# tum-vision/skeletondiffusion

Measured on AMD Instinct MI355X. Metric: generated futures/sec (AMASS 16-joint, 50 futures, T=100) at 1/2/4/8 GPUs, higher is better.
Workload: dtype f32 (emulated: 3 x f16 split products); 1 GPU; AMASS 16-joint nonisotropic sampling, T=100, 50 futures, batch=64 (config 2); J=16, T=100, sequences_per_gpu=64, sequences_total=64, futures=50, rows_per_gpu=3200, latent_dim=96, hipgraph=True, parallelism=dp1 (sequence-sharded, no data-path collective), row_chains=3, route=tiled split (k_gl4t + k_gl4 MODE 2/3), route_bits=24, kernel_variant=0

## Files before the change

### skeletondiffusion_amd/build.py

```python
from __future__ import annotations

import os
import shutil
import subprocess
import sys

HERE = os.path.dirname(os.path.abspath(__file__))
CSRC = os.path.join(HERE, "csrc")
OUT = os.path.join(HERE, "libskeldiff.so")
SOURCES = ["sd_kernels.hip", "sd_graph_linear.hip", "sd_graph_linear_v3.hip", "sd_graph_linear_v4.hip", "sd_graph_linear_v5.hip",
           "sd_metrics.hip", "sd_realism.hip", "sd_fid.hip", "sd_mmgt.hip", "sd_decoder.hip", "sd_train.hip", "sd_gru_train.hip",
           "sd_optim.hip", "sd_motion_batch.hip", "sd_q_sample.hip", "sd_plan.hip"]
HEADERS = ["sd_internal.h", "sd_gl4_args.h", "sd_realism_addr.h", "sd_gru_gates.h", "sd_optim_math.h", "sd_optim_table.h",
           "sd_philox.h", "sd_motion_batch_addr.h", "sd_q_sample_addr.h",
           os.path.join("..", "..", "include", "skeldiff.h")]


def _hipcc() -> str:
    for cand in (os.environ.get("HIPCC"), shutil.which("hipcc"), "/opt/rocm/bin/hipcc"):
        if cand and os.path.exists(cand):
            return cand
    raise RuntimeError("hipcc not found")


def _stale(stamp: str) -> bool:
    if not os.path.exists(OUT) or not os.path.exists(OUT + ".flags"):
        return True
    with open(OUT + ".flags") as f:
        if f.read() != stamp:
            return True
    t = os.path.getmtime(OUT)
    return any(os.path.getmtime(os.path.join(CSRC, f)) > t for f in SOURCES + HEADERS)


DEVICE_FLAGS = ["-Xclang", "-target-feature", "-Xclang", "-packed-fp32-ops"]
_FEATURE_NOTE = b"'-packed-fp32-ops' is not a recognized feature for this target"


def build_library(force: bool = False, verbose: bool = False, extra=(), tag="_dbg",
                  packed_fp32: bool = False) -> str:
    variant = bool(extra) or packed_fp32
    if packed_fp32 and tag == "_dbg":
        tag = "_packed"
    out = OUT.replace(".so", tag + ".so") if variant else OUT
    flags = ["--offload-arch=gfx950", "-O3", "-std=c++17", "-fPIC", "-Wno-pass-failed"] + \
        ([] if packed_fp32 else DEVICE_FLAGS) + list(extra)
    stamp = " ".join(flags)
# ... 45 lines not shown
```

### skeletondiffusion_amd/csrc/sd_graph_linear_v4.hip

```cpp
#include <hip/hip_runtime.h>
#include <stdint.h>

#include <algorithm>
#include <cmath>

#include "sd_gl4_args.h"
#include "sd_internal.h"

namespace sd {

typedef float floatx4 __attribute__((ext_vector_type(4)));
typedef float floatx8 __attribute__((ext_vector_type(8)));
typedef float floatx16 __attribute__((ext_vector_type(16)));
typedef _Float16 halfx8 __attribute__((ext_vector_type(8)));
typedef __bf16 bf16x8 __attribute__((ext_vector_type(8)));
typedef __bf16 bf16x4 __attribute__((ext_vector_type(4)));

namespace {

typedef __attribute__((address_space(3))) void lds_void;

template <int N>
struct VmCnt4 {
    static_assert(N >= 0 && N < 64, "vmcnt range");
    static constexpr int imm = (N & 0xF) | (0x7 << 4) | (0xF << 8) | ((N >> 4) << 14);
};

__device__ __forceinline__ floatx4 g4(const float* p) { return *reinterpret_cast<const floatx4*>(p); }

__device__ __forceinline__ float tanh4(float x) {
    const float e = __builtin_amdgcn_exp2f(2.0f * 1.44269504088896341f * x);
    return 1.0f - 2.0f * __builtin_amdgcn_rcpf(e + 1.0f);
}

__device__ __forceinline__ int64_t blk_off(int64_t row, int node, int f, int J, int F) {
    return ((((row >> 5) * J + node) * (int64_t)F) << 5) + ((f >> 3) << 8) + (((f >> 2) & 1) << 7) +
           ((row & 31) << 2) + (f & 3);
}


__global__ void k_absmax(const float* __restrict__ w, int64_t n, unsigned* __restrict__ out) {
    unsigned m = 0;
    for (int64_t i = (int64_t)blockIdx.x * blockDim.x + threadIdx.x; i < n; i += (int64_t)gridDim.x * blockDim.x)
        m = max(m, __float_as_uint(fabsf(w[i])));
    for (int o = 32; o > 0; o >>= 1) m = max(m, (unsigned)__shfl_xor((int)m, o));
    if ((threadIdx.x & 63) == 0) atomicMax(out, m);
}

__global__ void k_split_w(const float* __restrict__ W, int ntypes, int N, int K, int nct, float scale,
                          _Float16* __restrict__ out) {
    const int nchunk = K >> 4;
    const int64_t total = (int64_t)ntypes * nchunk * nct * 64;
    for (int64_t g = (int64_t)blockIdx.x * blockDim.x + threadIdx.x; g < total; g += (int64_t)gridDim.x * blockDim.x) {
// ... 75 lines not shown
    out->nct = ((N + 31) / 32 + 5) / 6 * 6;
    const int64_t n = (int64_t)ntypes * N * K;
    unsigned* dmax = nullptr;
    unsigned hmax = 0;
    hipError_t e = hipMalloc(&dmax, sizeof(unsigned));
    if (e != hipSuccess) return e;
    if ((e = hipMemsetAsync(dmax, 0, sizeof(unsigned), s)) != hipSuccess) return e;
    hipLaunchKernelGGL(k_absmax, dim3(256), dim3(256), 0, s, W, n, dmax);
    if ((e = hipGetLastError()) != hipSuccess) return e;
    if ((e = hipMemcpyAsync(&hmax, dmax, sizeof(unsigned), hipMemcpyDeviceToHost, s)) != hipSuccess) return e;
    if ((e = hipStreamSynchronize(s)) != hipSuccess) return e;
    (void)hipFree(dmax);
    const float amax = __builtin_bit_cast(float, hmax);
    int ex = 0;
    if (amax > 0.f && amax == amax && amax < 3.0e38f) (void)frexpf(amax, &ex);
    out->scale = ldexpf(1.0f, 15 - ex);
    out->unscale = ldexpf(1.0f, ex - 15);
    const size_t halves = (size_t)ntypes * (K / 16) * out->nct * 1024;
    if ((e = hipMalloc(&out->w, halves * sizeof(_Float16))) != hipSuccess) return e;
    const int64_t total = (int64_t)ntypes * (K / 16) * out->nct * 64;
    const int blocks = (int)std::min<int64_t>((total + 255) / 256, 4096);
    hipLaunchKernelGGL(k_split_w, dim3(blocks), dim3(256), 0, s, W, ntypes, N, K, out->nct, out->scale, out->w);
    return hipGetLastError();
}

struct YDst {
    float* y;
    int64_t y_rs, y_js, y_ts, y_cs;
};
struct YOut {
    GL4GArgs g;
};
static_assert(sizeof(YOut) == sizeof(GL4GArgs), "YOut: the GEMM-phase block");
__device__ __forceinline__ int64_t zs_off(int64_t row, int j, int n, int J, int N) {
    return ((((row >> 5) * (N >> 5) + (n >> 5)) * J + j) << 10) + ((row & 31) << 5) + (n & 31);
}

__device__ __forceinline__ floatx16 exact_tile_f32_impl(const float* x1, int64_t x1_rs, int K1, int x1_div,
                                                                  int64_t x1_row0, int x1_blk, const float* x2,
                                                                  int64_t x2_rs, int K2, int x2_blk, int64_t B, int J,
                                                                  const float* W, int wrow, int N, float unscale,
                                                                  int64_t row0, int j, int col0) {
    const int lane = threadIdx.x & 63, l32 = lane & 31, h = lane >> 5;
    const int K = K1 + K2;
    const int col = col0 + l32;
    const float* wr = W + (int64_t)(wrow + (col < N ? col : 0)) * K + 4 * h;
    const int64_t row = row0 + l32, ac = row < B ? row : 0;
    const float* xr1 = x1 + (x1_blk ? blk_off(row, j, 4 * h, J, K1) : ((ac + x1_row0) / x1_div) * x1_rs + (int64_t)j * K1 + 4 * h);
    const float* xr2 = !K2 ? xr1 : x2 + (x2_blk ? blk_off(row, j, 4 * h, J, K2) : ac * x2_rs + (int64_t)j * K2 + 4 * h);
    floatx16 c;
#pragma unroll
    for (int e = 0; e < 16; ++e) c[e] = 0.f;
#pragma nounroll
    for (int k0 = 0; k0 < K; k0 += 8) {
        const float* xp = k0 < K1 ? xr1 + (x1_blk ? (k0 >> 3) * 256 : k0) : xr2 + (x2_blk ? ((k0 - K1) >> 3) * 256 : k0 - K1);
        const float4 xv = *reinterpret_cast<const float4*>(xp);
        float4 wv = *reinterpret_cast<const float4*>(wr + k0);
        if (col >= N) wv = float4{0.f, 0.f, 0.f, 0.f};
        c = __builtin_amdgcn_mfma_f32_32x32x2f32(xv.x, wv.x, c, 0, 0, 0);
        c = __builtin_amdgcn_mfma_f32_32x32x2f32(xv.y, wv.y, c, 0, 0, 0);
        c = __builtin_amdgcn_mfma_f32_32x32x2f32(xv.z, wv.z, c, 0, 0, 0);
        c = __builtin_amdgcn_mfma_f32_32x32x2f32(xv.w, wv.w, c, 0, 0, 0);
    }
    const float up = 1.0f / unscale;
#pragma unroll
    for (int e = 0; e < 16; ++e) c[e] *= up;
    return c;
}
__device__ __forceinline__ floatx16 exact_tile_f32(const GLArgs& p, int64_t row0, int j, int col0) {
    return exact_tile_f32_impl(p.x1, p.x1_rs, p.K1, p.x1_div, p.x1_row0, p.x1_blk, p.x2, p.x2_rs, p.K2, p.x2_blk, p.B,
                               p.J, p.W, p.wrow[j], p.N, p.wsp_unscale, row0, j, col0);
}

__device__ __forceinline__ void gl4g_preload(const GL4GArgs& p) {
    asm volatile("" ::"s"(p.da.d), "s"(p.da.m), "s"(p.db.d), "s"(p.db.m), "s"(p.q8), "s"(p.r8), "s"(p.J), "s"(p.N), "s"(p.wsp),
                 "s"(p.x1), "s"(p.x2), "s"(p.bias), "s"(p.B), "s"(p.ntile_r), "s"(p.K1), "s"(p.K2), "s"(p.wsp_nct), "s"(p.pair_n),
                 "s"((int)p.x1_blk), "s"((int)p.x2_blk), "s"(p.x1_div));
    asm volatile("" ::"s"(p.ntype4[0]), "s"(p.ntype4[1]), "s"(p.ntype4[2]), "s"(p.ntype4[3]), "s"(p.ntype4[4]), "s"(p.ntype4[5]),
                 "s"(p.ntype4[6]), "s"(p.ntype4[7]), "s"(p.ntype4[8]), "s"(p.ntype4[9]), "s"(p.ntype4[10]), "s"(p.ntype4[11]),
                 "s"(p.ntype4[12]), "s"(p.ntype4[13]), "s"(p.ntype4[14]), "s"(p.ntype4[15]));
}

template <bool RMS, int PREC, bool ROWMAJOR, int PF = 8>
__global__ __launch_bounds__(256) void k_gl4y(const GL4GArgs p) {
    gl4g_preload(p);
    const int lane = threadIdx.x & 63, l32 = lane & 31, h = lane >> 5;
    const int wave = __builtin_amdgcn_readfirstlane(threadIdx.x >> 6);
    const Unit3 un = decode_unit(blockIdx.x * 4u + (uint32_t)wave, p.da, p.db);
    const int tc = (int)un.lo, j = (int)un.mid;
    const int64_t tr = un.hi;
    const int J = p.J;
    if (tr >= p.ntile_r) return;
    const int jt = gl4_node_type(p, j);
    const int64_t row0 = tr * 32;
    const int K = p.K1 + p.K2;
// ... 9 lines not shown

    floatx4 xa[PF], xb[PF];
    halfx8 wh[PF], wl[PF];
    auto issue = [&](int c, int sl) {
        const int k0 = c << 4;
        const float* src;
        int step4;
        if (k0 < p.K1) {
            src = p.x1_blk ? x1r + (k0 << 5) : x1r + k0;
            step4 = p.x1_blk ? 128 : 4;
        } else {
            src = p.x2_blk ? x2r + ((k0 - p.K1) << 5) : x2r + (k0 - p.K1);
            step4 = p.x2_blk ? 128 : 4;
        }
        xa[sl] = g4(src);
        xb[sl] = g4(src + step4);
        const _Float16* w = wbase + c * wcs;
        wh[sl] = *reinterpret_cast<const halfx8*>(w);
        if constexpr (!PREC) wl[sl] = *reinterpret_cast<const halfx8*>(w + 512);
    };
    floatx16 acc;
#pragma unroll
    for (int e = 0; e < 16; ++e) acc[e] = 0.f;
    float ss = 0.f, amx = 0.f;
    auto compute = [&](int c, int sl) {
        const floatx8 f = {xa[sl].x, xa[sl].y, xa[sl].z, xa[sl].w, xb[sl].x, xb[sl].y, xb[sl].z, xb[sl].w};
        if (RMS && (c << 4) < p.K1) {
            const floatx8 q = f * f;
            ss += ((q[0] + q[1]) + (q[2] + q[3])) + ((q[4] + q[5]) + (q[6] + q[7]));
        }
        const floatx8 a = __builtin_elementwise_abs(f);
        amx = fmaxf(amx, fmaxf(fmaxf(fmaxf(a[0], a[1]), fmaxf(a[2], a[3])), fmaxf(fmaxf(a[4], a[5]), fmaxf(a[6], a[7]))));
        const halfx8 xh = __builtin_convertvector(f, halfx8);
        acc = __builtin_amdgcn_mfma_f32_32x32x16_f16(xh, wh[sl], acc, 0, 0, 0);
        if constexpr (!PREC) {
            const halfx8 xl = __builtin_convertvector(f - __builtin_convertvector(xh, floatx8), halfx8);
            acc = __builtin_amdgcn_mfma_f32_32x32x16_f16(xh, wl[sl], acc, 0, 0, 0);
            acc = __builtin_amdgcn_mfma_f32_32x32x16_f16(xl, wh[sl], acc, 0, 0, 0);
        }
    };
    const int ncol = tc * 32 + l32;
    const float bv = (p.bias && ncol < p.N) ? p.bias[jt * p.N + ncol] : 0.f;
#pragma unroll
    for (int i = 0; i < PF; ++i) issue(i, i);
    for (int c0 = 0; c0 < nchunk - PF; c0 += PF) {
#pragma unroll
        for (int i = 0; i < PF; ++i) {
            compute(c0 + i, i);
            issue(c0 + i + PF, i);
        }
    }
#pragma unroll
    for (int i = 0; i < PF; ++i) compute(nchunk - PF + i, i);
    const bool oor = __builtin_amdgcn_ballot_w64(arow < p.B && amx >= 65504.0f) != 0;
    float sc[16];
#pragma unroll
    for (int r = 0; r < 16; ++r) sc[r] = p.wsp_unscale;
    if (RMS) {
        const float t = ss + __shfl_xor(ss, 32);
#pragma unroll
        for (int r = 0; r < 16; ++r) {
            const float n2 = __shfl(t, (r & 3) + 8 * (r >> 2) + 4 * h);
            sc[r] *= 1.0f / fmaxf(sqrtf(n2), 1e-12f);
        }
    }
    auto store = [&](const floatx16& v) {
        if constexpr (ROWMAJOR) {
            if (ncol < p.N) {
                float* y = p.y + tr * p.y_ts + (int64_t)j * p.y_js + (int64_t)tc * p.y_cs + l32;
#pragma unroll
                for (int r = 0; r < 16; ++r) {
                    const int rr = (r & 3) + 8 * (r >> 2) + 4 * h;
                    if (row0 + rr < p.B) y[(int64_t)rr * p.y_rs] = v[r] * sc[r] + bv;
                }
            }
        } else {
            float* y = p.y + tr * p.y_ts + (int64_t)j * p.y_js + (int64_t)tc * p.y_cs + l32;
#pragma unroll
            for (int r = 0; r < 16; ++r) y[((r & 3) + 8 * (r >> 2) + 4 * h) << 5] = v[r] * sc[r] + bv;
        }
    };
    store(acc);
    if (oor) {
        if (p.status && lane == 0) atomicOr(p.status, 1u);
        store(exact_tile_f32_impl(p.x1, p.x1_rs, p.K1, p.x1_div, p.x1_row0, p.x1_blk, p.x2, p.x2_rs, p.K2, p.x2_blk, p.B, p.J,
                                  p.W, jt * p.N, p.N, p.wsp_unscale, row0, j, tc * 32));
    }
}

template <int PREC, int CT, int NCH, int PF>
constexpr int gl4t_smem_bytes() {
    constexpr int TILE_H = PREC ? 512 : 1024, TS = 36, NWV = 4, NS = PF + 1;
    constexpr int SBW = NS * CT * TILE_H * 2;
    return SBW > NWV * 32 * TS * 4 ? SBW : NWV * 32 * TS * 4;
}

__device__ __forceinline__ void g4_async(floatx4& d, const float* p) {
    asm volatile("global_load_dwordx4 %0, %1, off" : "=v"(d) : "v"(p) : "memory");
}

template <bool RMS, int PREC, int CT, int NCH, bool ROWMAJOR, int RT, int PF>
__device__ __forceinline__ void gl4t_body(const GL4GArgs& p, const Unit3 un, const int tid, char* __restrict__ smem_raw) {
    static_assert(PREC != 2 || RT == 1, "bf16 operands: one row tile per wave");
    static_assert(PF >= 2 && PF <= 4, "chunks in flight");
    constexpr int NWV = 4;
    constexpr int NT = NWV * 64;
    constexpr int TILE_H = PREC ? 512 : 1024;
    constexpr int PPT = TILE_H / 8;
    constexpr int TS = 36;
    constexpr int NS = PF + 1;
    constexpr bool XV = PREC != 2;
    _Float16(*sW)[CT * TILE_H] = reinterpret_cast<_Float16(*)[CT * TILE_H]>(smem_raw);
    const int lane = tid & 63, l32 = lane & 31, h = lane >> 5;
    const int wave = __builtin_amdgcn_readfirstlane(tid >> 6);
    const int J = p.J;
    const int cg = (int)un.lo, ncg = (int)p.da.d;
    const int64_t ntile_r = p.ntile_r;
    const bool second = p.pair_n && 2 * cg >= ncg;
    const float unscale = second ? p.wsp_unscale2 : p.wsp_unscale;
    const int j = (int)un.hi;
    const int jt = gl4_node_type(p, j);
    const int64_t rgi = un.mid;
    const int64_t tr0 = (rgi * NWV + wave) * RT;
    int64_t row0[RT], arow[RT];
    const float* x1r[RT];
    const float* x2r[RT];
#pragma unroll
    for (int rt = 0; rt < RT; ++rt) {
        row0[rt] = (tr0 + rt < ntile_r ? tr0 + rt : 0) * 32;
        arow[rt] = row0[rt] + l32;
        const int64_t ac = arow[rt] < p.B ? arow[rt] : 0;
        x1r[rt] = p.x1_blk ? p.x1 + blk_off(arow[rt], j, 8 * h, J, p.K1)
                           : p.x1 + ((ac + p.x1_row0) / p.x1_div) * p.x1_rs + (int64_t)j * p.K1 + 8 * h;
        x2r[rt] = !p.K2 ? x1r[rt]
                        : p.x2_blk ? p.x2 + blk_off(arow[rt], j, 8 * h, J, p.K2) : p.x2 + ac * p.x2_rs + (int64_t)j * p.K2 + 8 * h;
    }
    const int c1 = p.K1 >> 4;
    const int cs1 = p.x1_blk ? 512 : 16, cs2 = p.x2_blk ? 512 : 16;
    const int st1 = p.x1_blk ? 128 : 4, st2 = p.x2_blk ? 128 : 4;
    const float* xp[RT];
#pragma unroll
    for (int rt = 0; rt < RT; ++rt) xp[rt] = c1 > 0 ? x1r[rt] : x2r[rt];
    auto xstep = [&](int c) { return c < c1 ? st1 : st2; };
    floatx4 xa[NS][RT], xb[NS][RT];
    floatx16 acc[RT][CT];
#pragma unroll
    for (int rt = 0; rt < RT; ++rt)
#pragma unroll
        for (int ct = 0; ct < CT; ++ct)
#pragma unroll
            for (int e = 0; e < 16; ++e) acc[rt][ct][e] = 0.f;
    float ss[RT], amx[RT];
#pragma unroll
    for (int rt = 0; rt < RT; ++rt) ss[rt] = amx[rt] = 0.f;
    float bvp[CT];
#pragma unroll
    for (int ct = 0; ct < CT; ++ct) bvp[ct] = p.bias ? p.bias[jt * p.N + (cg * CT + ct) * 32 + l32] : 0.f;
    const _Float16* wt0 = p.wsp + ((int64_t)jt * NCH * p.wsp_nct + cg * CT) * 1024;
    constexpr int NPC = CT * PPT;
    constexpr int XL = 2 * RT;
    constexpr int OPA = (NPC / 64 + NWV - 1) / NWV + XL, OPB = (NPC / 64) / NWV + XL;
    static_assert(OPA * (PF - 1) < 64, "vmcnt range");
    const bool wa = wave * 64 + NT * ((NPC / 64 + NWV - 1) / NWV - 1) < NPC;
    auto fill = [&](int c) {
        _Float16* dst = sW[c % NS];
#pragma unroll
        for (int k = 0; k < (NPC / 64 + NWV - 1) / NWV; ++k) {
            const int q0 = wave * 64 + NT * k;
            if (q0 >= NPC) continue;
            const int q = q0 + lane;
            const _Float16* src = wt0 + ((int64_t)c * p.wsp_nct + q / PPT) * 1024 + (q % PPT) * 8;
            __builtin_amdgcn_global_load_lds((const void*)src, (lds_void*)(dst + (size_t)q0 * 8), 16, 0, 0);
        }
        const int s = c % NS;
#pragma unroll
        for (int rt = 0; rt < RT; ++rt) {
            const float* src = xp[rt];
            xp[rt] = c + 1 == c1 ? x2r[rt] : src + (c < c1 ? cs1 : cs2);
            if constexpr (XV) {
                g4_async(xa[s][rt], src);
                g4_async(xb[s][rt], src + xstep(c));
            } else {
                const bool bsrc = c < c1 ? p.x1_bf16 : p.x2_bf16;
                const float* base = c < c1 ? p.x1 : p.x2;
                const float* qb = reinterpret_cast<const float*>(reinterpret_cast<const __bf16*>(base) + (src - base));
                xa[s][rt] = g4(bsrc ? qb : src);
                xb[s][rt] = g4(bsrc ? qb : src + xstep(c));
            }
        }
    };
    auto compute = [&](int c) {
        const int s = c % NS;
        const _Float16* wt = sW[s] + lane * 8;
        const bool rms_chunk = RMS && c < c1;
        if constexpr (PREC == 2) {
            const bool bsrc = c < c1 ? p.x1_bf16 : p.x2_bf16;
            bf16x8 xb16;
            floatx8 f;
            if (bsrc) {
                xb16 = __builtin_bit_cast(bf16x8, xa[s][0]);
                f = __builtin_convertvector(xb16, floatx8);
            } else {
                f = floatx8{xa[s][0].x, xa[s][0].y, xa[s][0].z, xa[s][0].w, xb[s][0].x, xb[s][0].y, xb[s][0].z, xb[s][0].w};
                xb16 = __builtin_convertvector(f, bf16x8);
            }
            if (rms_chunk) {
                const floatx8 q = f * f;
                ss[0] += ((q[0] + q[1]) + (q[2] + q[3])) + ((q[4] + q[5]) + (q[6] + q[7]));
            }
#pragma unroll
            for (int ct = 0; ct < CT; ++ct) {
                const bf16x8 wb = *reinterpret_cast<const bf16x8*>(wt + ct * TILE_H);
                acc[0][ct] = __builtin_amdgcn_mfma_f32_32x32x16_bf16(xb16, wb, acc[0][ct], 0, 0, 0);
            }
            return;
        }
        halfx8 xh[RT], xl[RT];
#pragma unroll
        for (int rt = 0; rt < RT; ++rt) {
            const floatx8 f = {xa[s][rt].x, xa[s][rt].y, xa[s][rt].z, xa[s][rt].w,
                               xb[s][rt].x, xb[s][rt].y, xb[s][rt].z, xb[s][rt].w};
            if (rms_chunk) {
                const floatx8 q = f * f;
                ss[rt] += ((q[0] + q[1]) + (q[2] + q[3])) + ((q[4] + q[5]) + (q[6] + q[7]));
            }
            const floatx8 a = __builtin_elementwise_abs(f);
            amx[rt] = fmaxf(amx[rt], fmaxf(fmaxf(fmaxf(a[0], a[1]), fmaxf(a[2], a[3])), fmaxf(fmaxf(a[4], a[5]), fmaxf(a[6], a[7]))));
            xh[rt] = __builtin_convertvector(f, halfx8);
            if constexpr (!PREC) xl[rt] = __builtin_convertvector(f - __builtin_convertvector(xh[rt], floatx8), halfx8);
            asm volatile("" : "+v"(amx[rt]), "+v"(ss[rt]));
        }
#pragma unroll
        for (int ct = 0; ct < CT; ++ct) {
            const halfx8 wh = *reinterpret_cast<const halfx8*>(wt + ct * TILE_H);
            halfx8 wl;
            if constexpr (!PREC) wl = *reinterpret_cast<const halfx8*>(wt + ct * TILE_H + 512);
#pragma unroll
            for (int rt = 0; rt < RT; ++rt) {
                floatx16 t = __builtin_amdgcn_mfma_f32_32x32x16_f16(xh[rt], wh, acc[rt][ct], 0, 0, 0);
                if constexpr (!PREC) {
                    t = __builtin_amdgcn_mfma_f32_32x32x16_f16(xh[rt], wl, t, 0, 0, 0);
                    t = __builtin_amdgcn_mfma_f32_32x32x16_f16(xl[rt], wh, t, 0, 0, 0);
                }
                acc[rt][ct] = t;
            }
        }
    };
    auto wait_chunk = [&](int c, int younger) {
        switch (younger) {
            case 0: __builtin_amdgcn_s_waitcnt(VmCnt4<0>::imm & ~(0xF << 8)); break;
            case 1:
                if (wa) __builtin_amdgcn_s_waitcnt(VmCnt4<OPA>::imm & ~(0xF << 8));
                else __builtin_amdgcn_s_waitcnt(VmCnt4<OPB>::imm & ~(0xF << 8));
                break;
            case 2:
                if (wa) __builtin_amdgcn_s_waitcnt(VmCnt4<2 * OPA>::imm & ~(0xF << 8));
                else __builtin_amdgcn_s_waitcnt(VmCnt4<2 * OPB>::imm & ~(0xF << 8));
                break;
            default:
                if (wa) __builtin_amdgcn_s_waitcnt(VmCnt4<3 * OPA>::imm & ~(0xF << 8));
                else __builtin_amdgcn_s_waitcnt(VmCnt4<3 * OPB>::imm & ~(0xF << 8));
                break;
        }
        if constexpr (XV) {
#pragma unroll
            for (int rt = 0; rt < RT; ++rt) asm volatile("" : "+v"(xa[c % NS][rt]), "+v"(xb[c % NS][rt]) :: "memory");
        }
        asm volatile("" ::: "memory");
        __builtin_amdgcn_s_barrier();
        asm volatile("" ::: "memory");
    };
    static_assert(NCH >= PF, "ring depth");
#pragma unroll
    for (int i = 0; i < PF; ++i) fill(i);
#pragma unroll
    for (int c = 0; c < NCH; ++c) {
        wait_chunk(c, NCH - 1 - c < PF - 1 ? NCH - 1 - c : PF - 1);
        if constexpr (XV) {
            if (c + PF < NCH) fill(c + PF);
            asm volatile("" ::: "memory");
            compute(c);
        } else {
            compute(c);
            asm volatile("" ::: "memory");
            if (c + PF < NCH) fill(c + PF);
        }
        asm volatile("" ::: "memory");
    }
    __syncthreads();
    float* sT = reinterpret_cast<float*>(smem_raw) + wave * 32 * TS;
#pragma unroll
    for (int rt = 0; rt < RT; ++rt) {
        const int64_t tr = tr0 + rt;
        if (tr >= ntile_r) break;
        const bool oor = PREC != 2 && __builtin_amdgcn_ballot_w64(arow[rt] < p.B && amx[rt] >= 65504.0f) != 0;
        float sc[16];
#pragma unroll
        for (int r = 0; r < 16; ++r) sc[r] = unscale;
        if (RMS) {
            const float t = ss[rt] + __shfl_xor(ss[rt], 32);
#pragma unroll
            for (int r = 0; r < 16; ++r) {
                const float n2 = __shfl(t, (r & 3) + 8 * (r >> 2) + 4 * h);
                sc[r] *= 1.0f / fmaxf(sqrtf(n2), 1e-12f);
            }
        }
        float* y = p.y + tr * p.y_ts + (int64_t)j * p.y_js + (int64_t)cg * CT * p.y_cs;
        auto store_tile = [&](int ct, const floatx16& v, float bv) {
#pragma unroll
            for (int r = 0; r < 16; ++r) sT[((r & 3) + 8 * (r >> 2) + 4 * h) * TS + l32] = v[r] * sc[r] + bv;
            __builtin_amdgcn_wave_barrier();
#pragma unroll
            for (int q = 0; q < 4; ++q) {
                const int row = 8 * q + (lane >> 3), c4 = (lane & 7) * 4;
                const floatx4 o = *reinterpret_cast<const floatx4*>(sT + row * TS + c4);
                if (!ROWMAJOR || row0[rt] + row < p.B)
                    *reinterpret_cast<floatx4*>(y + (int64_t)row * p.y_rs + (int64_t)ct * p.y_cs + c4) = o;
            }
            __builtin_amdgcn_wave_barrier();
        };
#pragma unroll
        for (int ct = 0; ct < CT; ++ct) store_tile(ct, acc[rt][ct], bvp[ct]);
        if (oor) {
            if (p.status && lane == 0) atomicOr(p.status, 1u);
#pragma nounroll
            for (int ct = 0; ct < CT; ++ct) {
                const int col = (cg * CT + ct) * 32;
                const floatx16 ex = exact_tile_f32_impl(p.x1, p.x1_rs, p.K1, p.x1_div, p.x1_row0, p.x1_blk, p.x2, p.x2_rs, p.K2,
                                                        p.x2_blk, p.B, p.J, second ? p.W2 : p.W,
                                                        jt * (p.pair_n ? p.pair_n : p.N), p.pair_n ? p.pair_n : p.N,
                                                        unscale, row0[rt], j, second ? col - p.pair_n : col);
                store_tile(ct, ex, p.bias ? p.bias[jt * p.N + col + l32] : 0.f);
            }
        }
    }
}

template <bool RMS, int PREC, int CT, int NCH, bool ROWMAJOR, int RT, int PF>
__global__ __launch_bounds__(256, 2) void k_gl4t(const GLArgs, int, int64_t, const YOut yo) {
    __shared__ __attribute__((aligned(16))) char smem_raw[gl4t_smem_bytes<PREC, CT, NCH, PF>()];
    const GL4GArgs& p = yo.g;
    gl4g_preload(p);
    const Unit3 un = decode_unit(xcd_remap(blockIdx.x, p.q8, p.r8), p.da, p.db);
    gl4t_body<RMS, PREC, CT, NCH, ROWMAJOR, RT, PF>(p, un, threadIdx.x, smem_raw);
}

template <int J, int NW, int NPW, bool FROM_YS = false, class A = GLArgs>
__device__ __forceinline__ void attention_epilogue(const A& p, floatx16 (&acc)[NPW][1][3], float* smem,
                                                   const float* sG, int64_t row0, int head, int wave, int lane,
                                                   int q8only = 0) {
    constexpr int COLS = 96;
    constexpr int JT = (J + 15) / 16;
    constexpr int KS = (J + 3) / 4;
    constexpr int YS8 = 8 * COLS + 16;
    constexpr int ZN = 100;
    constexpr int ZR = J * ZN;
    const int l32 = lane & 31, h = lane >> 5, lr = lane & 15, lg = lane >> 4;
    const int hid = p.attn_heads * 32;
    float* sY = smem;
    float* sZ = FROM_YS ? smem : smem + J * YS8;
    float ga[JT][KS];
#pragma unroll
    for (int it = 0; it < JT; ++it)
#pragma unroll
        for (int s = 0; s < KS; ++s) {
            const int i = 16 * it + lr, jj = 4 * s + lg;
            ga[it][s] = (i < J && jj < J) ? sG[i * J + jj] : 0.f;
        }
#pragma unroll
    for (int q8 = 0; q8 < 4; ++q8) {
        if (FROM_YS && q8 != q8only) continue;
        if constexpr (!FROM_YS) {
            __syncthreads();
// ... 258 lines not shown
            if (kk >= kcount) continue;
            const int k = kfirst + kk;
            const int b = k < BPW ? wave + NW * k : COLS;
            int r, cc;
            out_pos(min(b, COLS - 1), r, cc);
            const int64_t row = row0 + 16 * hc + r;
            const int n = c0 + cc;
            const bool ok = b < COLS && row < p.B && n < p.N;
#pragma unroll
            for (int ib = 0; ib < IB; ++ib) {
                const int i = ib * 16 + lr;
                const int64_t ro = p.res_blk ? blk_off(row, i, n, J, p.N) : row * p.res_rs + (int64_t)i * p.N + n;
                if (PREC == 2 && p.res_bf16)
                    rv[kk][ib] = (ok && i < J) ? __builtin_convertvector(
                                                     *reinterpret_cast<const bf16x4*>(reinterpret_cast<const __bf16*>(p.res) + ro), floatx4)
                                               : floatx4{0.f, 0.f, 0.f, 0.f};
                else
                    rv[kk][ib] = (ok && i < J) ? g4(p.res + ro) : floatx4{0.f, 0.f, 0.f, 0.f};
            }
        }
    };

    floatx16 acc[NPW][RT][CT];
    if constexpr (PH2) {
        constexpr int C4 = COLS / 4;
        constexpr int YQ = MODE == 2 ? J * 16 * C4 : J * 8 * 24;
        constexpr int NYL = (YQ + NTH - 1) / NTH, NGL = (J * J + NTH - 1) / NTH;
        constexpr int YS8 = 8 * COLS + 16;
        const int64_t tb = (row0 >> 5) * J;
        (void)tb;
        auto ysrc = [&](int q, float*& dst) -> const float* {
            if constexpr (MODE == 2) {
                static_assert(MODE != 2 || COLS == 32, "MODE 2: one 32-column tile");
                const int cc = (q % C4) * 4, r = (q / C4) & 15, j = q / (16 * C4);
                dst = sY + j * YS + r * YR + cc;
                return p.zs + zs_off(row0 + 16 * slab + r, j, p.zs_c0 + c0 + cc, J, p.zs_n);
            } else {
                const int cc = (q & 7) * 4, rr = (q >> 3) & 7, j = (q >> 6) % J, ct = (q >> 6) / J;
                dst = sY + j * YS8 + rr * COLS + 32 * ct + cc;
                return p.zs + zs_off(row0 + 8 * slab + rr, j, (ctile + ct * p.attn_heads) * 32 + cc, J, p.N);
            }
        };
        floatx4 yv[NYL];
        float gv[NGL];
        float f0 = 1.0f, f1 = 0.0f;
#pragma unroll
        for (int k = 0; k < NYL; ++k) {
            const int q = tid + k * NTH;
            float* d;
            if (q < YQ) {
                yv[k] = g4(ysrc(q, d));
            }
        }
        if constexpr (MODE == 2 && RES_EARLY)
            if (p.res) load_res(slab, 0, BPW);
#pragma unroll
        for (int k = 0; k < NGL; ++k)
            if (tid + k * NTH < J * J) gv[k] = p.G[tid + k * NTH];
        if (tid < COLS && p.film && c0 + tid < p.N) {
            f0 = p.film[c0 + tid] + 1.0f;
            f1 = p.film[p.N + c0 + tid];
        }
#pragma unroll
        for (int k = 0; k < NYL; ++k) {
            const int q = tid + k * NTH;
            float* d;
            if (q < YQ) {
                (void)ysrc(q, d);
                *reinterpret_cast<floatx4*>(d) = yv[k];
            }
        }
// ... 512 lines not shown
    hipLaunchKernelGGL(kt, grid, block, 0, s, a, ncg, ntile_r, yd);
    return hipGetLastError();
}

template <bool ROWMAJOR>
static hipError_t launch_gl4t(const GLArgs& a, bool rms, int64_t ntile_r, const YDst& yo, hipStream_t s) {
    const int K = a.K1 + a.K2;
    if (a.K1 % 16 || (a.x1_div != 1 && a.x1_blk)) return hipErrorNotSupported;
    if (ROWMAJOR && a.N % 256 == 0 && K == 192 && a.prec != 2) return launch_gl4t_v<8, 12, ROWMAJOR, 1>(a, rms, ntile_r, yo, s);
    constexpr bool kRt2 = true;
    constexpr int kPf = 2, kPf6 = 2;
    constexpr int PFB = ROWMAJOR ? 2 : kPf, PF6 = ROWMAJOR ? 2 : kPf6;
    const int Nt = a.pair_n ? a.pair_n : a.N;
    if (!ROWMAJOR && kRt2 && a.prec != 2 && Nt <= 192 && Nt % 96 == 0) {
        if (K == 192) return launch_gl4t_v<3, 12, ROWMAJOR, 2, PFB>(a, rms, ntile_r, yo, s);
        if (K == 256) return launch_gl4t_v<3, 16, ROWMAJOR, 2, PFB>(a, rms, ntile_r, yo, s);
        if (K == 384) return launch_gl4t_v<3, 24, ROWMAJOR, 2, PFB>(a, rms, ntile_r, yo, s);
    }
    if (Nt % 192 == 0) {
        if (K == 192) return launch_gl4t_v<6, 12, ROWMAJOR, 1, PF6>(a, rms, ntile_r, yo, s);
        if (K == 256) return launch_gl4t_v<6, 16, ROWMAJOR, 1, PF6>(a, rms, ntile_r, yo, s);
        if (K == 384) return launch_gl4t_v<6, 24, ROWMAJOR, 1, PF6>(a, rms, ntile_r, yo, s);
    } else if (Nt % 96 == 0) {
        if (K == 192) return launch_gl4t_v<3, 12, ROWMAJOR, 1>(a, rms, ntile_r, yo, s);
        if (K == 384) return launch_gl4t_v<3, 24, ROWMAJOR, 1>(a, rms, ntile_r, yo, s);
    }
    return hipErrorNotSupported;
}

template <int J>
static hipError_t gl4_split(const GLArgs& a, bool rms, bool attn, int route, hipStream_t s) {
    const int64_t ntile_r = (a.B + 31) / 32;
    const int ntc = a.N / 32;
    const YDst yo{a.zs, 32, 1024, (int64_t)(a.N / 32) * J * 1024, (int64_t)J * 1024};
    hipError_t e = route == 2 ? launch_gl4t<false>(a, rms, ntile_r, yo, s) : hipErrorNotSupported;
    if (e == hipErrorNotSupported) {
        if (a.prec == 2) return hipErrorNotSupported;
        e = launch_gl4y<false>(a, rms, ntc, ntile_r, yo, s);
    }
    if (e != hipSuccess) return e;
    if (a.prec == 2) {
        if (attn) return gl4_launch_t<J, 8, 1, 3, 3, 2, 0>(a, false, s);
        return gl4_launch_t<J, 8, 1, 1, 2, 2, 0>(a, false, s);
    }
    if (attn) return gl4_launch_t<J, 8, 1, 3, 3, 0, 0>(a, false, s);
    return gl4_launch_t<J, 8, 1, 1, 2, 0, 0>(a, false, s);
}

static hipError_t gl4_split_dispatch(const GLArgs& a, bool rms, bool attn, int route, hipStream_t s) {
    switch (a.J) {
        case 16: return gl4_split<16>(a, rms, attn, route, s);
        case 17: return gl4_split<17>(a, rms, attn, route, s);
        case 21: return gl4_split<21>(a, rms, attn, route, s);
        default: return hipErrorNotSupported;
    }
}

template <int J>
static hipError_t gl4_pair(const GLArgs& pr, const GLArgs& a, const GLArgs& b, hipStream_t s) {
    const int64_t ntile_r = (pr.B + 31) / 32;
    const YDst yo{pr.zs, 32, 1024, (int64_t)(pr.N / 32) * J * 1024, (int64_t)J * 1024};
    const hipError_t e = launch_gl4t<false>(pr, false, ntile_r, yo, s);
    if (e != hipSuccess) return e;
    if (!gl4_grid_ok((int64_t)(a.N + b.N) / 32 * ntile_r * 2)) return hipErrorInvalidValue;
    const dim3 grid((unsigned)((a.N + b.N) / 32 * ntile_r * 2));
    GL4PairArgs pp;
    if (!pack_gl4_pair(a, b, &pp)) return hipErrorInvalidValue;
    const size_t lds = ((size_t)J * (16 * 36 + 16) + (size_t)J * J + 64) * sizeof(float);
    static_assert((J * (16 * 36 + 16) + J * J + 64) * sizeof(float) <= 64 * 1024, "default dynamic LDS");
    g_route_bits |= kRouteMixPhase;
    if (pr.prec == 2) hipLaunchKernelGGL((k_gl4_pair<J, 2>), grid, dim3(512), lds, s, pp);
    else hipLaunchKernelGGL((k_gl4_pair<J, 0>), grid, dim3(512), lds, s, pp);
    return hipGetLastError();
}

bool graph_linear_pair_ok(const GLArgs& pr, const GLArgs& a, const GLArgs& b) {
    if (a.J != 16 && a.J != 17 && a.J != 21) return false;
    const int K = a.K1 + a.K2;
    if (!pr.wsp || !a.wsp || !b.wsp || !pr.pair_n || a.N != pr.pair_n || b.N != pr.pair_n || pr.N != 2 * pr.pair_n ||
        pr.wsp_nct * 32 != pr.N || a.N % 192 || (K != 192 && K != 384))
        return false;
    for (const GLArgs* g : {&a, &b}) {
        if (((uintptr_t)g->out & 15) || ((uintptr_t)g->res & 15) || (g->res && (g->res_rs & 3)) || (g->out_rs & 3)) return false;
        if (g->x1 != pr.x1 || g->x2 != pr.x2 || g->K1 != pr.K1 || g->K2 != pr.K2 || g->B != pr.B || g->zs != pr.zs ||
            g->x1_div != pr.x1_div || g->x1_row0 != pr.x1_row0 || g->x1_blk != pr.x1_blk || g->x2_blk != pr.x2_blk ||
            g->x1_bf16 != pr.x1_bf16 || g->x2_bf16 != pr.x2_bf16 || g->prec != pr.prec || g->zs_n != pr.N)
            return false;
    }
    if (a.zs_c0 != 0 || b.zs_c0 != a.N) return false;
    if (K % 32 || a.K1 % 16 || (a.x1_blk && a.x1_div != 1)) return false;
    return split_route(a, false) == 2 && split_route(b, false) == 2 && split_route(pr, false) == 2;
}

hipError_t launch_graph_linear_pair_v4(const GLArgs& pr, const GLArgs& a, const GLArgs& b, hipStream_t s) {
// ... 92 lines not shown
```

Before: 17190 futures/s.

## Swap MFMA operands and re-tile zs layout for direct vectorized epilogue stores

```diff
diff --git a/skeletondiffusion_amd/build.py b/skeletondiffusion_amd/build.py
--- a/skeletondiffusion_amd/build.py
+++ b/skeletondiffusion_amd/build.py
@@ -12,7 +12,7 @@
            "sd_metrics.hip", "sd_realism.hip", "sd_fid.hip", "sd_mmgt.hip", "sd_decoder.hip", "sd_train.hip", "sd_gru_train.hip",
            "sd_optim.hip", "sd_motion_batch.hip", "sd_q_sample.hip", "sd_plan.hip"]
 HEADERS = ["sd_internal.h", "sd_gl4_args.h", "sd_realism_addr.h", "sd_gru_gates.h", "sd_optim_math.h", "sd_optim_table.h",
-           "sd_philox.h", "sd_motion_batch_addr.h", "sd_q_sample_addr.h",
+           "sd_philox.h", "sd_motion_batch_addr.h", "sd_q_sample_addr.h", "sd_ystore_map.h",
            os.path.join("..", "..", "include", "skeldiff.h")]
 
 
diff --git a/skeletondiffusion_amd/csrc/sd_graph_linear_v4.hip b/skeletondiffusion_amd/csrc/sd_graph_linear_v4.hip
--- a/skeletondiffusion_amd/csrc/sd_graph_linear_v4.hip
+++ b/skeletondiffusion_amd/csrc/sd_graph_linear_v4.hip
@@ -6,6 +6,7 @@
 
 #include "sd_gl4_args.h"
 #include "sd_internal.h"
+#include "sd_ystore_map.h"
 
 namespace sd {
 
@@ -19,6 +20,8 @@
 namespace {
 
 typedef __attribute__((address_space(3))) void lds_void;
+typedef __attribute__((address_space(3))) float lds_float;
+typedef __attribute__((address_space(3))) floatx4 lds_floatx4;
 
 template <int N>
 struct VmCnt4 {
@@ -160,10 +163,8 @@
     GL4GArgs g;
 };
 static_assert(sizeof(YOut) == sizeof(GL4GArgs), "YOut: the GEMM-phase block");
-__device__ __forceinline__ int64_t zs_off(int64_t row, int j, int n, int J, int N) {
-    return ((((row >> 5) * (N >> 5) + (n >> 5)) * J + j) << 10) + ((row & 31) << 5) + (n & 31);
-}
-
+
+template <bool SWAP = false>
 __device__ __forceinline__ floatx16 exact_tile_f32_impl(const float* x1, int64_t x1_rs, int K1, int x1_div,
                                                                   int64_t x1_row0, int x1_blk, const float* x2,
                                                                   int64_t x2_rs, int K2, int x2_blk, int64_t B, int J,
@@ -185,10 +186,17 @@
         const float4 xv = *reinterpret_cast<const float4*>(xp);
         float4 wv = *reinterpret_cast<const float4*>(wr + k0);
         if (col >= N) wv = float4{0.f, 0.f, 0.f, 0.f};
-        c = __builtin_amdgcn_mfma_f32_32x32x2f32(xv.x, wv.x, c, 0, 0, 0);
-        c = __builtin_amdgcn_mfma_f32_32x32x2f32(xv.y, wv.y, c, 0, 0, 0);
-        c = __builtin_amdgcn_mfma_f32_32x32x2f32(xv.z, wv.z, c, 0, 0, 0);
-        c = __builtin_amdgcn_mfma_f32_32x32x2f32(xv.w, wv.w, c, 0, 0, 0);
+        if constexpr (SWAP) {
+            c = __builtin_amdgcn_mfma_f32_32x32x2f32(wv.x, xv.x, c, 0, 0, 0);
+            c = __builtin_amdgcn_mfma_f32_32x32x2f32(wv.y, xv.y, c, 0, 0, 0);
+            c = __builtin_amdgcn_mfma_f32_32x32x2f32(wv.z, xv.z, c, 0, 0, 0);
+            c = __builtin_amdgcn_mfma_f32_32x32x2f32(wv.w, xv.w, c, 0, 0, 0);
+        } else {
+            c = __builtin_amdgcn_mfma_f32_32x32x2f32(xv.x, wv.x, c, 0, 0, 0);
+            c = __builtin_amdgcn_mfma_f32_32x32x2f32(xv.y, wv.y, c, 0, 0, 0);
+            c = __builtin_amdgcn_mfma_f32_32x32x2f32(xv.z, wv.z, c, 0, 0, 0);
+            c = __builtin_amdgcn_mfma_f32_32x32x2f32(xv.w, wv.w, c, 0, 0, 0);
+        }
     }
     const float up = 1.0f / unscale;
 #pragma unroll
@@ -264,11 +272,11 @@
         const floatx8 a = __builtin_elementwise_abs(f);
         amx = fmaxf(amx, fmaxf(fmaxf(fmaxf(a[0], a[1]), fmaxf(a[2], a[3])), fmaxf(fmaxf(a[4], a[5]), fmaxf(a[6], a[7]))));
         const halfx8 xh = __builtin_convertvector(f, halfx8);
-        acc = __builtin_amdgcn_mfma_f32_32x32x16_f16(xh, wh[sl], acc, 0, 0, 0);
+        acc = __builtin_amdgcn_mfma_f32_32x32x16_f16(wh[sl], xh, acc, 0, 0, 0);
         if constexpr (!PREC) {
             const halfx8 xl = __builtin_convertvector(f - __builtin_convertvector(xh, floatx8), halfx8);
-            acc = __builtin_amdgcn_mfma_f32_32x32x16_f16(xh, wl[sl], acc, 0, 0, 0);
-            acc = __builtin_amdgcn_mfma_f32_32x32x16_f16(xl, wh[sl], acc, 0, 0, 0);
+            acc = __builtin_amdgcn_mfma_f32_32x32x16_f16(wl[sl], xh, acc, 0, 0, 0);
+            acc = __builtin_amdgcn_mfma_f32_32x32x16_f16(wh[sl], xl, acc, 0, 0, 0);
         }
     };
     const int ncol = tc * 32 + l32;
@@ -282,49 +290,55 @@
             issue(c0 + i + PF, i);
         }
     }
+    __shared__ __attribute__((aligned(16))) float sBy[4 * 32];
+    float* sB = sBy + wave * 32;
+    sB[l32] = bv;
 #pragma unroll
     for (int i = 0; i < PF; ++i) compute(nchunk - PF + i, i);
     const bool oor = __builtin_amdgcn_ballot_w64(arow < p.B && amx >= 65504.0f) != 0;
-    float sc[16];
-#pragma unroll
-    for (int r = 0; r < 16; ++r) sc[r] = p.wsp_unscale;
+    float sc = p.wsp_unscale;
     if (RMS) {
         const float t = ss + __shfl_xor(ss, 32);
-#pragma unroll
-        for (int r = 0; r < 16; ++r) {
-            const float n2 = __shfl(t, (r & 3) + 8 * (r >> 2) + 4 * h);
-            sc[r] *= 1.0f / fmaxf(sqrtf(n2), 1e-12f);
-        }
-    }
+        sc *= 1.0f / fmaxf(sqrtf(t), 1e-12f);
+    }
+    const bool vec = !ROWMAJOR || ((((uintptr_t)p.y) & 15) == 0 && (p.y_rs & 3) == 0 && (p.N & 3) == 0);
     auto store = [&](const floatx16& v) {
-        if constexpr (ROWMAJOR) {
-            if (ncol < p.N) {
-                float* y = p.y + tr * p.y_ts + (int64_t)j * p.y_js + (int64_t)tc * p.y_cs + l32;
-#pragma unroll
-                for (int r = 0; r < 16; ++r) {
-                    const int rr = (r & 3) + 8 * (r >> 2) + 4 * h;
-                    if (row0 + rr < p.B) y[(int64_t)rr * p.y_rs] = v[r] * sc[r] + bv;
-                }
-            }
-        } else {
-            float* y = p.y + tr * p.y_ts + (int64_t)j * p.y_js + (int64_t)tc * p.y_cs + l32;
-#pragma unroll
-            for (int r = 0; r < 16; ++r) y[((r & 3) + 8 * (r >> 2) + 4 * h) << 5] = v[r] * sc[r] + bv;
+        if (ROWMAJOR && arow >= p.B) return;
+        float* y = p.y + tr * p.y_ts + (int64_t)j * p.y_js + (int64_t)tc * p.y_cs +
+                   (ROWMAJOR ? ystore_rm_piece_off(l32, h, 0, p.y_rs) : ystore_zs_piece_off(l32, h, 0));
+#pragma unroll
+        for (int g = 0; g < 4; ++g) {
+            const floatx4 b4 = *reinterpret_cast<const floatx4*>(sB + ystore_col(g, h));
+            floatx4 o;
+#pragma unroll
+            for (int e = 0; e < 4; ++e) o[e] = v[4 * g + e] * sc + b4[e];
+            const int col = tc * 32 + ystore_col(g, h);
+            if (vec) {
+                if (!ROWMAJOR) *reinterpret_cast<floatx4*>(y + ystore_zs_piece_off(0, 0, g)) = o;
+                else if (col < p.N) *reinterpret_cast<floatx4*>(y + ystore_col(g, 0)) = o;
+            } else {
+#pragma unroll
+                for (int e = 0; e < 4; ++e)
+                    if (col + e < p.N) y[ystore_col(g, 0) + e] = o[e];
+            }
         }
     };
     store(acc);
     if (oor) {
         if (p.status && lane == 0) atomicOr(p.status, 1u);
-        store(exact_tile_f32_impl(p.x1, p.x1_rs, p.K1, p.x1_div, p.x1_row0, p.x1_blk, p.x2, p.x2_rs, p.K2, p.x2_blk, p.B, p.J,
-                                  p.W, jt * p.N, p.N, p.wsp_unscale, row0, j, tc * 32));
-    }
-}
-
-template <int PREC, int CT, int NCH, int PF>
+        store(exact_tile_f32_impl<true>(p.x1, p.x1_rs, p.K1, p.x1_div, p.x1_row0, p.x1_blk, p.x2, p.x2_rs, p.K2, p.x2_blk, p.B,
+                                        p.J, p.W, jt * p.N, p.N, p.wsp_unscale, row0, j, tc * 32));
+    }
+}
+
+template <int PREC, int CT, int PF, bool ROWMAJOR>
+constexpr int gl4t_ring_bytes() {
+    constexpr int TILE_H = PREC ? 512 : 1024, NWV = 4, NS = PF + 1, TR = NWV * 32 * 36 * 4;
+    return !ROWMAJOR || NS * CT * TILE_H * 2 > TR ? NS * CT * TILE_H * 2 : TR;
+}
+template <int PREC, int CT, int NCH, int PF, bool ROWMAJOR>
 constexpr int gl4t_smem_bytes() {
-    constexpr int TILE_H = PREC ? 512 : 1024, TS = 36, NWV = 4, NS = PF + 1;
-    constexpr int SBW = NS * CT * TILE_H * 2;
-    return SBW > NWV * 32 * TS * 4 ? SBW : NWV * 32 * TS * 4;
+    return gl4t_ring_bytes<PREC, CT, PF, ROWMAJOR>() + 4 * CT * 32 * 4;
 }
 
 __device__ __forceinline__ void g4_async(floatx4& d, const float* p) {
@@ -339,10 +353,13 @@
     constexpr int NT = NWV * 64;
     constexpr int TILE_H = PREC ? 512 : 1024;
     constexpr int PPT = TILE_H / 8;
-    constexpr int TS = 36;
     constexpr int NS = PF + 1;
     constexpr bool XV = PREC != 2;
     _Float16(*sW)[CT * TILE_H] = reinterpret_cast<_Float16(*)[CT * TILE_H]>(smem_raw);
+    float* sB = reinterpret_cast<float*>(smem_raw + gl4t_ring_bytes<PREC, CT, PF, ROWMAJOR>()) + (tid >> 6) * (CT * 32);
+    lds_float* sBw = (lds_float*)(sB + (tid & 31));
+    const lds_floatx4* sBr = (const lds_floatx4*)(sB + 4 * ((tid >> 5) & 1));
+    asm volatile("" : "+v"(sBw), "+v"(sBr));
     const int lane = tid & 63, l32 = lane & 31, h = lane >> 5;
     const int wave = __builtin_amdgcn_readfirstlane(tid >> 6);
     const int J = p.J;
@@ -387,7 +404,10 @@
     for (int rt = 0; rt < RT; ++rt) ss[rt] = amx[rt] = 0.f;
     float bvp[CT];
 #pragma unroll
-    for (int ct = 0; ct < CT; ++ct) bvp[ct] = p.bias ? p.bias[jt * p.N + (cg * CT + ct) * 32 + l32] : 0.f;
+    for (int ct = 0; ct < CT; ++ct) {
+        const float* bsrc = p.bias ? p.bias + jt * p.N + (cg * CT + ct) * 32 + l32 : reinterpret_cast<const float*>(p.wsp);
+        asm volatile("global_load_dword %0, %1, off" : "=v"(bvp[ct]) : "v"(bsrc) : "memory");
+    }
     const _Float16* wt0 = p.wsp + ((int64_t)jt * NCH * p.wsp_nct + cg * CT) * 1024;
     constexpr int NPC = CT * PPT;
     constexpr int XL = 2 * RT;
@@ -443,7 +463,7 @@
 #pragma unroll
             for (int ct = 0; ct < CT; ++ct) {
                 const bf16x8 wb = *reinterpret_cast<const bf16x8*>(wt + ct * TILE_H);
-                acc[0][ct] = __builtin_amdgcn_mfma_f32_32x32x16_bf16(xb16, wb, acc[0][ct], 0, 0, 0);
+                acc[0][ct] = __builtin_amdgcn_mfma_f32_32x32x16_bf16(wb, xb16, acc[0][ct], 0, 0, 0);
             }
             return;
         }
@@ -469,10 +489,10 @@
             if constexpr (!PREC) wl = *reinterpret_cast<const halfx8*>(wt + ct * TILE_H + 512);
 #pragma unroll
             for (int rt = 0; rt < RT; ++rt) {
-                floatx16 t = __builtin_amdgcn_mfma_f32_32x32x16_f16(xh[rt], wh, acc[rt][ct], 0, 0, 0);
+                floatx16 t = __builtin_amdgcn_mfma_f32_32x32x16_f16(wh, xh[rt], acc[rt][ct], 0, 0, 0);
                 if constexpr (!PREC) {
-                    t = __builtin_amdgcn_mfma_f32_32x32x16_f16(xh[rt], wl, t, 0, 0, 0);
-                    t = __builtin_amdgcn_mfma_f32_32x32x16_f16(xl[rt], wh, t, 0, 0, 0);
+                    t = __builtin_amdgcn_mfma_f32_32x32x16_f16(wl, xh[rt], t, 0, 0, 0);
+                    t = __builtin_amdgcn_mfma_f32_32x32x16_f16(wh, xl[rt], t, 0, 0, 0);
                 }
                 acc[rt][ct] = t;
             }
@@ -508,6 +528,13 @@
 #pragma unroll
     for (int c = 0; c < NCH; ++c) {
         wait_chunk(c, NCH - 1 - c < PF - 1 ? NCH - 1 - c : PF - 1);
+        if (c == 0) {
+#pragma unroll
+            for (int ct = 0; ct < CT; ++ct) {
+                asm volatile("" : "+v"(bvp[ct]));
+                sBw[ct * 32] = p.bias ? bvp[ct] : 0.f;
+            }
+        }
         if constexpr (XV) {
             if (c + PF < NCH) fill(c + PF);
             asm volatile("" ::: "memory");
@@ -519,50 +546,54 @@
         }
         asm volatile("" ::: "memory");
     }
-    __syncthreads();
+    constexpr int TS = 36;
     float* sT = reinterpret_cast<float*>(smem_raw) + wave * 32 * TS;
+    if constexpr (ROWMAJOR) __syncthreads();
 #pragma unroll
     for (int rt = 0; rt < RT; ++rt) {
         const int64_t tr = tr0 + rt;
         if (tr >= ntile_r) break;
         const bool oor = PREC != 2 && __builtin_amdgcn_ballot_w64(arow[rt] < p.B && amx[rt] >= 65504.0f) != 0;
-        float sc[16];
-#pragma unroll
-        for (int r = 0; r < 16; ++r) sc[r] = unscale;
+        float sc = unscale;
         if (RMS) {
             const float t = ss[rt] + __shfl_xor(ss[rt], 32);
-#pragma unroll
-            for (int r = 0; r < 16; ++r) {
-                const float n2 = __shfl(t, (r & 3) + 8 * (r >> 2) + 4 * h);
-                sc[r] *= 1.0f / fmaxf(sqrtf(n2), 1e-12f);
-            }
-        }
-        float* y = p.y + tr * p.y_ts + (int64_t)j * p.y_js + (int64_t)cg * CT * p.y_cs;
-        auto store_tile = [&](int ct, const floatx16& v, float bv) {
-#pragma unroll
-            for (int r = 0; r < 16; ++r) sT[((r & 3) + 8 * (r >> 2) + 4 * h) * TS + l32] = v[r] * sc[r] + bv;
-            __builtin_amdgcn_wave_barrier();
-#pragma unroll
-            for (int q = 0; q < 4; ++q) {
-                const int row = 8 * q + (lane >> 3), c4 = (lane & 7) * 4;
-                const floatx4 o = *reinterpret_cast<const floatx4*>(sT + row * TS + c4);
-                if (!ROWMAJOR || row0[rt] + row < p.B)
-                    *reinterpret_cast<floatx4*>(y + (int64_t)row * p.y_rs + (int64_t)ct * p.y_cs + c4) = o;
-            }
-            __builtin_amdgcn_wave_barrier();
+            sc *= 1.0f / fmaxf(sqrtf(t), 1e-12f);
+        }
+        float* y = p.y + tr * p.y_ts + (int64_t)j * p.y_js + (int64_t)cg * CT * p.y_cs + (ROWMAJOR ? 0 : ystore_zs_piece_off(l32, h, 0));
+        auto store_tile = [&](int ct, const floatx16& v) {
+#pragma unroll
+            for (int g = 0; g < 4; ++g) {
+                const floatx4 bv = sBr[(ct * 32 + ystore_col(g, 0)) / 4];
+                floatx4 o;
+#pragma unroll
+                for (int e = 0; e < 4; ++e) o[e] = v[4 * g + e] * sc + bv[e];
+                if constexpr (ROWMAJOR) *reinterpret_cast<floatx4*>(sT + l32 * TS + ystore_col(g, h)) = o;
+                else *reinterpret_cast<floatx4*>(y + (int64_t)ct * p.y_cs + ystore_zs_piece_off(0, 0, g)) = o;
+            }
+            if constexpr (ROWMAJOR) {
+                __builtin_amdgcn_wave_barrier();
+#pragma unroll
+                for (int q = 0; q < 4; ++q) {
+                    const int row = 8 * q + (lane >> 3), c4 = (lane & 7) * 4;
+                    const floatx4 o = *reinterpret_cast<const floatx4*>(sT + row * TS + c4);
+                    if (row0[rt] + row < p.B)
+                        *reinterpret_cast<floatx4*>(y + (int64_t)row * p.y_rs + (int64_t)ct * p.y_cs + c4) = o;
+                }
+                __builtin_amdgcn_wave_barrier();
+            }
         };
 #pragma unroll
-        for (int ct = 0; ct < CT; ++ct) store_tile(ct, acc[rt][ct], bvp[ct]);
+        for (int ct = 0; ct < CT; ++ct) store_tile(ct, acc[rt][ct]);
         if (oor) {
             if (p.status && lane == 0) atomicOr(p.status, 1u);
 #pragma nounroll
             for (int ct = 0; ct < CT; ++ct) {
                 const int col = (cg * CT + ct) * 32;
-                const floatx16 ex = exact_tile_f32_impl(p.x1, p.x1_rs, p.K1, p.x1_div, p.x1_row0, p.x1_blk, p.x2, p.x2_rs, p.K2,
-                                                        p.x2_blk, p.B, p.J, second ? p.W2 : p.W,
-                                                        jt * (p.pair_n ? p.pair_n : p.N), p.pair_n ? p.pair_n : p.N,
-                                                        unscale, row0[rt], j, second ? col - p.pair_n : col);
-                store_tile(ct, ex, p.bias ? p.bias[jt * p.N + col + l32] : 0.f);
+                const floatx16 ex = exact_tile_f32_impl<true>(p.x1, p.x1_rs, p.K1, p.x1_div, p.x1_row0, p.x1_blk, p.x2, p.x2_rs,
+                                                              p.K2, p.x2_blk, p.B, p.J, second ? p.W2 : p.W,
+                                                              jt * (p.pair_n ? p.pair_n : p.N), p.pair_n ? p.pair_n : p.N,
+                                                              unscale, row0[rt], j, second ? col - p.pair_n : col);
+                store_tile(ct, ex);
             }
         }
     }
@@ -570,7 +601,7 @@
 
 template <bool RMS, int PREC, int CT, int NCH, bool ROWMAJOR, int RT, int PF>
 __global__ __launch_bounds__(256, 2) void k_gl4t(const GLArgs, int, int64_t, const YOut yo) {
-    __shared__ __attribute__((aligned(16))) char smem_raw[gl4t_smem_bytes<PREC, CT, NCH, PF>()];
+    __shared__ __attribute__((aligned(16))) char smem_raw[gl4t_smem_bytes<PREC, CT, NCH, PF, ROWMAJOR>()];
     const GL4GArgs& p = yo.g;
     gl4g_preload(p);
     const Unit3 un = decode_unit(xcd_remap(blockIdx.x, p.q8, p.r8), p.da, p.db);
@@ -895,11 +926,15 @@
         auto ysrc = [&](int q, float*& dst) -> const float* {
             if constexpr (MODE == 2) {
                 static_assert(MODE != 2 || COLS == 32, "MODE 2: one 32-column tile");
-                const int cc = (q % C4) * 4, r = (q / C4) & 15, j = q / (16 * C4);
+                const int j = q / (16 * C4);
+                int cc, r;
+                zs_slab_piece(q % (16 * C4), 16, &r, &cc);
                 dst = sY + j * YS + r * YR + cc;
                 return p.zs + zs_off(row0 + 16 * slab + r, j, p.zs_c0 + c0 + cc, J, p.zs_n);
             } else {
-                const int cc = (q & 7) * 4, rr = (q >> 3) & 7, j = (q >> 6) % J, ct = (q >> 6) / J;
+                const int j = (q >> 6) % J, ct = (q >> 6) / J;
+                int cc, rr;
+                zs_slab_piece(q & 63, 8, &rr, &cc);
                 dst = sY + j * YS8 + rr * COLS + 32 * ct + cc;
                 return p.zs + zs_off(row0 + 8 * slab + rr, j, (ctile + ct * p.attn_heads) * 32 + cc, J, p.N);
             }
@@ -1478,7 +1513,8 @@
 static hipError_t gl4_split(const GLArgs& a, bool rms, bool attn, int route, hipStream_t s) {
     const int64_t ntile_r = (a.B + 31) / 32;
     const int ntc = a.N / 32;
-    const YDst yo{a.zs, 32, 1024, (int64_t)(a.N / 32) * J * 1024, (int64_t)J * 1024};
+    const ZsStrides zst = zs_strides(J, a.N);
+    const YDst yo{a.zs, 0, zst.y_js, zst.y_ts, zst.y_cs};
     hipError_t e = route == 2 ? launch_gl4t<false>(a, rms, ntile_r, yo, s) : hipErrorNotSupported;
     if (e == hipErrorNotSupported) {
         if (a.prec == 2) return hipErrorNotSupported;
@@ -1505,7 +1541,8 @@
 template <int J>
 static hipError_t gl4_pair(const GLArgs& pr, const GLArgs& a, const GLArgs& b, hipStream_t s) {
     const int64_t ntile_r = (pr.B + 31) / 32;
-    const YDst yo{pr.zs, 32, 1024, (int64_t)(pr.N / 32) * J * 1024, (int64_t)J * 1024};
+    const ZsStrides zst = zs_strides(J, pr.N);
+    const YDst yo{pr.zs, 0, zst.y_js, zst.y_ts, zst.y_cs};
     const hipError_t e = launch_gl4t<false>(pr, false, ntile_r, yo, s);
     if (e != hipSuccess) return e;
     if (!gl4_grid_ok((int64_t)(a.N + b.N) / 32 * ntile_r * 2)) return hipErrorInvalidValue;
diff --git a/skeletondiffusion_amd/csrc/sd_ystore_map.h b/skeletondiffusion_amd/csrc/sd_ystore_map.h
--- /dev/null
+++ b/skeletondiffusion_amd/csrc/sd_ystore_map.h
@@ -0,0 +1,33 @@
+#pragma once
+#include <stdint.h>
+
+#if defined(__HIPCC__)
+#define SD_YS_HD __host__ __device__ __forceinline__
+#else
+#define SD_YS_HD inline
+#endif
+
+namespace sd {
+
+SD_YS_HD int ystore_col(int g, int h) { return 8 * g + 4 * h; }
+
+SD_YS_HD int ystore_zs_piece_off(int l32, int h, int g) { return g * 256 + l32 * 8 + 4 * h; }
+SD_YS_HD int64_t ystore_rm_piece_off(int l32, int h, int g, int64_t y_rs) { return (int64_t)l32 * y_rs + ystore_col(g, h); }
+
+SD_YS_HD int zs_blk_off(int r, int c) { return ((c >> 3) << 8) + (r << 3) + (c & 7); }
+
+SD_YS_HD int64_t zs_off(int64_t row, int j, int n, int J, int N) {
+    return ((((row >> 5) * (N >> 5) + (n >> 5)) * J + j) << 10) + zs_blk_off((int)(row & 31), n & 31);
+}
+
+SD_YS_HD void zs_slab_piece(int t, int R, int* r, int* c) {
+    *c = (t / (2 * R)) * 8 + (t & 1) * 4;
+    *r = (t % (2 * R)) >> 1;
+}
+
+struct ZsStrides {
+    int64_t y_js, y_ts, y_cs;
+};
+SD_YS_HD ZsStrides zs_strides(int J, int N) { return ZsStrides{1024, (int64_t)(N / 32) * J * 1024, (int64_t)J * 1024}; }
+
+}
```

Result: faster. 17450 futures/s, median of 6 (+1.5%).
